# jbush001/RustNetworkStack

Measured on AMD Instinct MI355X. Metric: GiB/s device-resident Internet checksum, 1500B-packet batches, 1/2/4/8 GPUs, higher is better.
Workload: dtype u8

## Files before the change

### rustnetworkstack_amd/csrc/k_packed.hip

```cpp
#include "rns_launch.hpp"

#ifndef RNS_ROWS_DEEP_FROM
#define RNS_ROWS_DEEP_FROM 1024u
#endif
#ifndef RNS_TX_ROWS_DEEP_FROM
#define RNS_TX_ROWS_DEEP_FROM 1024u
#endif
#ifndef RNS_RX_ROWS_D
#define RNS_RX_ROWS_D 8
#endif

namespace rns {

constexpr bool kStreamNT = RNS_STREAM_NT != 0;

template <class Kernel>
static int launch_rows(const CsumArgs &a, uint32_t deep_from, hipStream_t st, Kernel kernel)
{
    return with_flags(
        [&](auto deep, auto buf) {
            return launch(kernel(std::integral_constant<int, deep() ? 16 : 8>{}, buf), dim3(waves64(a.n)), dim3(64), 0,
                          st, a);
        },
        a.len_hint >= deep_from, buf_ok(a));
}

int launch_stream_rx(const CsumArgs &a, hipStream_t st)
{
    return with_flags(
        [&](auto ack, auto buf) {
            if constexpr (ack())
                return launch(csum_stream_kernel<kStreamNT, buf()>, dim3(waves64(a.n)), dim3(64), 0, st, a);
            else
                return launch(csum_rows_rx_kernel<kStreamNT, buf(), RNS_RX_ROWS_D>, dim3(waves64(a.n)), dim3(64), 0, st,
                              a);
        },
        a.arena_bytes / a.n <= 128, buf_ok(a));
}

int dispatch_packed(const CsumArgs &a, const Shape &sh, hipStream_t st)
{
    const bool tiny = (sh.variant & ~16u) == 3u && sh.G == 4u && sh.U == 1u;
    if (a.align_mask >= 15u && !tiny)
        return launch_rows(a, RNS_ROWS_DEEP_FROM, st,
                           [](auto D, auto buf) { return csum_rows_kernel<kStreamNT, buf(), D()>; });
    const bool mixed = (sh.variant & 4u) != 0;
    if (!mixed && !tiny)
        return RNS_E_INVALID;
    const uint64_t batches = waves64(a.n);
    const uint64_t wpb = (mixed ? kMixedBlock<false> : kBlock) / 64;
    uint64_t blocks = (batches + wpb - 1) / wpb;
    if (sh.max_blocks != 0 && blocks > sh.max_blocks)
        blocks = sh.max_blocks;
    const dim3 grid(static_cast<uint32_t>(blocks)), block(mixed ? kMixedBlock<false> : kBlock);
    if (mixed)
        return with_flags(
            [&](auto nt, auto buf) {
                return launch(csum_mixed_kernel<false, nt(), buf(), false, false, false, true>, grid, block, 0, st, a);
            },
            (sh.variant & 2u) != 0, buf_ok(a));
    return with_flags(
        [&](auto buf, auto pf) {
            return launch(csum_rounds_kernel<4, 1, false, true, buf(), 1, true, pf()>, grid, block, 0, st, a);
        },
        buf_ok(a), (sh.variant & 16u) != 0);
}

int launch_fill_packed(const CsumArgs &a, hipStream_t st)
{
    return launch_rows(a, RNS_ROWS_DEEP_FROM, st,
                       [](auto D, auto buf) { return csum_rows_kernel<kStreamNT, buf(), D(), true>; });
}

int launch_tx_packed(const CsumArgs &a, hipStream_t st)
{
    return launch_rows(a, RNS_TX_ROWS_DEEP_FROM, st,
                       [](auto D, auto buf) { return csum_rows_tx_kernel<kStreamNT, buf(), D()>; });
}

int launch_strided_rx(const CsumArgs &a, hipStream_t st)
{
    constexpr int B = kStridedRxB;
    const dim3 grid(static_cast<uint32_t>((static_cast<uint64_t>(a.n) + 64 * B - 1) / (64 * B)));
    return with_flags([&](auto buf) { return launch(csum_strided_rx_kernel<buf(), B>, grid, dim3(64), 0, st, a); },
                      buf_ok(a));
}

// ... 2 lines not shown
```

### rustnetworkstack_amd/csrc/rns_checksum.hip

```cpp
#include <hip/hip_runtime.h>

#include <algorithm>
#include <cmath>
#include <cstdint>
#include <cstdio>

#include "rns_launch.hpp"

using namespace rns;

namespace {

__global__ __launch_bounds__(kBlock) void splitmix64_fill_kernel(uint8_t *buf, uint64_t nbytes, uint64_t seed)
{
    const uint64_t nwords = (nbytes + 7) / 8;
    const uint64_t stride = static_cast<uint64_t>(gridDim.x) * blockDim.x;
    for (uint64_t i = static_cast<uint64_t>(blockIdx.x) * blockDim.x + threadIdx.x; i < nwords; i += stride) {
        uint64_t z = seed + (i + 1) * 0x9E3779B97F4A7C15ull;
        z = (z ^ (z >> 30)) * 0xBF58476D1CE4E5B9ull;
        z = (z ^ (z >> 27)) * 0x94D049BB133111EBull;
        z = z ^ (z >> 31);
        if ((i + 1) * 8 <= nbytes) {
            reinterpret_cast<uint64_t *>(buf)[i] = z;
        } else {
// ... 115 lines not shown

#ifndef RNS_CHAIN_NT_FROM
#define RNS_CHAIN_NT_FROM 384u
#endif
bool chain_nt_from_hint(uint32_t frag_len_hint) { return (frag_len_hint ? frag_len_hint : 512u) >= RNS_CHAIN_NT_FROM; }
bool chain_nt_from_arena(uint64_t arena_bytes, uint32_t n_frags, double mean)
{
    const double frag_est = mean > 0.5 ? static_cast<double>(arena_bytes) / n_frags * (mean - 0.5) / mean : 0.0;
    return n_frags == 0 || frag_est >= RNS_CHAIN_NT_FROM;
}

bool chain_deep(uint32_t K, double mean) { return K >= 3 || (K == 2 && mean >= 2.0); }

template <bool FILL>
int chain_launch(CsumArgs &a, uint32_t frag_len_hint, hipStream_t stream)
{
    const double mean = chain_mean(a);
    a.chain_k = chain_pick_k(mean);
    if ((a.flags & RNS_FLAG_CHAIN_TX_PACKED) && mean <= 1.0 + kRunFrags)
        return launch_txrows<FILL>(a, stream);
    const bool runs = kChainRuns && (a.flags & RNS_FLAG_CHAIN_RUNS) && buf_ok(a);
    return launch_chain<FILL>(a, a.chain_k, chain_nt_from_hint(frag_len_hint), runs, chain_deep(a.chain_k, mean), stream);
}

constexpr uint64_t kRxGridCap = 4096;
dim3 stash_grid(uint64_t n, uint64_t arena_bytes, bool tiny_cap)
{
    constexpr int BLK = kMixedBlock<true>;
    uint64_t blocks = (waves64(n) + BLK / 64 - 1) / (BLK / 64);
    const bool cap = tiny_cap && arena_bytes / n <= 128;
    if (cap && blocks > kRxGridCap)
        blocks = kRxGridCap;
    return dim3(static_cast<uint32_t>(blocks));
}

bool misaligned(const void *p, uintptr_t mask) { return (reinterpret_cast<uintptr_t>(p) & mask) != 0; }

bool pool_rx_valid(const uint8_t *d_pool, uint32_t buf_log2, uint32_t min_log2, const uint32_t *d_buf_idx, uint32_t n_frags,
                   const uint32_t *d_blk_first, const uint16_t *d_len16, uint32_t n_pkts, const uint8_t *local_ipv4,
                   const uint8_t *local_ipv6, const uint8_t *d_status)
{
    return d_pool && buf_log2 >= min_log2 && buf_log2 <= kPoolMaxLog2 && d_blk_first && d_len16 && (!n_frags || d_buf_idx) &&
           n_pkts <= RNS_CHAIN_MAX_PACKETS && !misaligned(d_pool, 15) && rx_valid(d_status, local_ipv4, local_ipv6);
}

int pool_rx_verify(PoolRx &rx, bool &nt, const uint8_t *d_pool, uint64_t pool_bytes, uint32_t buf_log2,
                   const uint32_t *d_buf_idx, uint32_t n_frags, const uint32_t *d_blk_first, const uint16_t *d_len16,
                   uint32_t n_pkts, const uint8_t *local_ipv4, const uint8_t *local_ipv6, uint8_t *d_status, uint16_t *d_l4_sum,
                   void *stream)
{
    RNS_TRY(rns_rx_verify_pool_dev(d_pool, pool_bytes, buf_log2, d_buf_idx, n_frags, d_blk_first, d_len16, n_pkts, local_ipv4,
                                   local_ipv6, d_status, d_l4_sum, stream));
    rx = PoolRx{d_pool, pool_bytes, d_buf_idx, d_blk_first, d_len16, d_status, n_pkts, n_frags, buf_log2};
    nt = chain_nt_from_arena(pool_bytes, n_frags, static_cast<double>(n_frags) / n_pkts);
    return RNS_OK;
}

bool pool_tx_valid(const uint8_t *d_tx_pool, const uint32_t *d_free, uint32_t n_free, uint32_t cap, const uint32_t *d_ip_id_add,
                   const uint32_t *d_tx_blk_first, const uint8_t *d_tx_head_len8, const uint16_t *d_tx_pay_len16,
                   const uint32_t *d_tx_src, const uint32_t *d_count)
{
    return d_tx_pool && d_count && (!n_free || d_free) && (!cap || (d_tx_blk_first && d_tx_head_len8 && d_tx_pay_len16)) &&
           !misaligned(d_tx_pool, 15) && !misaligned(d_free, 3) && !misaligned(d_ip_id_add, 3) &&
           !misaligned(d_tx_blk_first, 3) && !misaligned(d_tx_pay_len16, 1) && !misaligned(d_tx_src, 3) &&
           !misaligned(d_count, 3);
}

void set_pool_tx(PoolTx &tx, uint8_t *d_tx_pool, uint64_t tx_pool_bytes, uint32_t buf_log2, const uint32_t *d_free,
                 uint32_t n_free, uint32_t cap, uint16_t ip_id_base, const uint32_t *d_ip_id_add, uint32_t *d_tx_blk_first,
                 uint8_t *d_tx_head_len8, uint16_t *d_tx_pay_len16, uint32_t *d_tx_src, uint32_t *d_count)
{
    tx = PoolTx{d_tx_pool, tx_pool_bytes >> buf_log2, d_free, d_ip_id_add, d_tx_blk_first, d_tx_head_len8, d_tx_pay_len16,
                d_tx_src, d_count, n_free, cap, ip_id_base, buf_log2};
}

int count_only(uint32_t *d_count, size_t bytes, void *stream)
{
    if (!d_count || misaligned(d_count, 3))
        return RNS_E_INVALID;
    RNS_TRY(check_device());
    return launch_fill32(d_count, bytes / 4, 0u, static_cast<hipStream_t>(stream));
}

}

extern "C" {

int rns_csum_batch_dev_cfg(const uint8_t *d_arena, uint64_t arena_bytes, const uint64_t *d_off,
                           const uint32_t *d_len, const uint16_t *d_seed, uint16_t *d_out, uint32_t n,
                           uint32_t flags, uint32_t variant, uint32_t lanes_per_packet, uint32_t unroll,
                           uint32_t max_blocks, uint32_t *d_bad, void *stream)
{
    return entry(n, d_off && d_len && d_out, d_arena, arena_bytes, flags, stream, [&](CsumArgs &a, hipStream_t st) {
        set_explicit(a, d_off, d_len);
        set_results(a, d_seed, d_out, d_bad);
        return dispatch<false>(a, variant, lanes_per_packet, unroll, max_blocks, st);
    });
}

int rns_csum_batch_dev(const uint8_t *d_arena, uint64_t arena_bytes, const uint64_t *d_off,
                       const uint32_t *d_len, const uint16_t *d_seed, uint16_t *d_out, uint32_t n,
                       uint32_t flags, uint32_t len_hint, uint32_t *d_bad, void *stream)
{
    const Shape sh = pick_shape(len_hint);
    return rns_csum_batch_dev_cfg(d_arena, arena_bytes, d_off, d_len, d_seed, d_out, n, flags, sh.variant, sh.G,
                                  sh.U, sh.max_blocks, d_bad, stream);
}

int rns_csum_batch_dev_off32(const uint8_t *d_arena, uint64_t arena_bytes, const uint32_t *d_off32,
                             const uint32_t *d_len, const uint16_t *d_seed, uint16_t *d_out, uint32_t n,
                             uint32_t flags, uint32_t len_hint, uint32_t *d_bad, void *stream)
{
    return entry(n, d_off32 && d_len && d_out, d_arena, arena_bytes, flags, stream, [&](CsumArgs &a, hipStream_t st) {
        a.off32 = d_off32;
        a.len = d_len;
        set_results(a, d_seed, d_out, d_bad);
        const Shape sh = pick_shape(len_hint);
        return dispatch<false>(a, sh.variant, sh.G, sh.U, sh.max_blocks, st);
    });
}

int rns_csum_batch_packed_dev(const uint8_t *d_arena, uint64_t arena_bytes, const uint64_t *d_blk_off,
                              const uint16_t *d_len16, uint32_t align_log2, const uint16_t *d_seed, uint16_t *d_out,
                              uint32_t n, uint32_t flags, uint32_t len_hint, uint32_t *d_bad, void *stream)
{
    return entry(n, d_blk_off && d_len16 && d_out && packed_align(align_log2, 0), d_arena, arena_bytes, flags, stream,
                 [&](CsumArgs &a, hipStream_t st) {
                     set_packed(a, d_blk_off, d_len16, align_log2);
                     set_results(a, d_seed, d_out, d_bad);
                     a.len_hint = len_hint;
                     Shape sh = pick_shape(len_hint);
                     if ((sh.variant & 5u) == 0)
                         sh = Shape{6u, 0u, 0u, 0u};
                     return dispatch_packed(a, sh, st);
                 });
}

int rns_csum_batch_strided_dev(const uint8_t *d_arena, uint64_t arena_bytes, uint64_t first_off,
                               uint64_t stride, uint32_t len, const uint16_t *d_seed, uint16_t *d_out,
                               uint32_t n, uint32_t flags, uint32_t *d_bad, void *stream)
{
    return entry(n, d_out && strided_fits(first_off, stride, n), d_arena, arena_bytes, flags, stream,
                 [&](CsumArgs &a, hipStream_t st) {
                     set_strided(a, first_off, stride);
                     set_results(a, d_seed, d_out, d_bad);
                     a.fixed_len = len;
                     if (len != 0 && len <= 64 && ((first_off + a.base_adjust) & 15) == 0 && (stride & 15) == 0)
                         return launch_strided_tiny(a, st);
                     const Shape sh = pick_shape(len);
                     return dispatch<true>(a, sh.variant, sh.G, sh.U, sh.max_blocks, st);
                 });
}

int rns_csum_chain_dev(const uint8_t *d_arena, uint64_t arena_bytes, const uint64_t *d_frag_off,
                       const uint32_t *d_frag_len, uint32_t n_frags, const uint32_t *d_first,
                       const uint16_t *d_seed, uint16_t *d_out, uint32_t n_pkts, uint32_t flags,
                       uint32_t frag_len_hint, uint16_t *d_frag_sums, uint32_t *d_bad, void *stream)
{
    (void)d_frag_sums;
    return entry(n_pkts, d_out && chain_valid(d_frag_off, d_frag_len, d_first, n_frags, n_pkts), d_arena, arena_bytes,
                 flags, stream, [&](CsumArgs &a, hipStream_t st) {
                     set_chain(a, d_frag_off, d_frag_len, d_first, n_frags);
                     set_results(a, d_seed, d_out, d_bad);
                     return chain_launch<false>(a, frag_len_hint, st);
                 });
}

int rns_csum_chain_fill_dev(uint8_t *d_arena, uint64_t arena_bytes, const uint64_t *d_frag_off,
                            const uint32_t *d_frag_len, uint32_t n_frags, const uint32_t *d_first,
                            const uint16_t *d_seed, const uint16_t *d_field, uint32_t field_off, uint16_t *d_out,
                            uint32_t n_pkts, uint32_t flags, uint32_t frag_len_hint, uint32_t *d_bad, void *stream)
{
    return entry(n_pkts, chain_valid(d_frag_off, d_frag_len, d_first, n_frags, n_pkts), d_arena, arena_bytes, flags,
                 stream, [&](CsumArgs &a, hipStream_t st) {
                     set_chain(a, d_frag_off, d_frag_len, d_first, n_frags);
                     set_results(a, d_seed, d_out, d_bad);
                     set_field(a, d_field, field_off);
                     return chain_launch<true>(a, frag_len_hint, st);
                 });
}

int rns_csum_fill_dev(uint8_t *d_arena, uint64_t arena_bytes, const uint64_t *d_off, const uint32_t *d_len,
                      const uint16_t *d_seed, const uint16_t *d_field, uint32_t field_off, uint16_t *d_out,
                      uint32_t n, uint32_t flags, uint32_t *d_bad, void *stream)
{
    return entry(n, d_off && d_len, d_arena, arena_bytes, flags, stream, [&](CsumArgs &a, hipStream_t st) {
        set_explicit(a, d_off, d_len);
        set_results(a, d_seed, d_out, d_bad);
        set_field(a, d_field, field_off);
        return launch_fill(a, stash_grid(n, arena_bytes, false), st);
    });
}

int rns_csum_fill_packed_dev(uint8_t *d_arena, uint64_t arena_bytes, const uint64_t *d_blk_off, const uint16_t *d_len16,
                             uint32_t align_log2, const uint16_t *d_seed, const uint16_t *d_field, uint32_t field_off,
                             uint16_t *d_out, uint32_t n, uint32_t flags, uint32_t len_hint, uint32_t *d_bad,
                             void *stream)
{
    return entry(n, d_blk_off && d_len16 && packed_align(align_log2, 4), d_arena, arena_bytes, flags, stream,
                 [&](CsumArgs &a, hipStream_t st) {
                     set_packed(a, d_blk_off, d_len16, align_log2);
// ... 475 lines not shown
                 d_head_blk_off && d_head_len8 && d_pay_blk_off && d_pay_len16 && packed_align(pay_align_log2, 4) &&
                     n <= RNS_CHAIN_MAX_PACKETS,
                 d_arena, arena_bytes, RNS_FLAG_COMPLEMENT, stream, [&](CsumArgs &a, hipStream_t st) {
                     a.head_blk_off = d_head_blk_off;
                     a.head_len8 = d_head_len8;
                     set_packed(a, d_pay_blk_off, d_pay_len16, pay_align_log2);
                     set_tx_status(a, d_status);
                     return launch_txrows<false, true, true>(a, st);
                 });
}

int rns_tx_fill_pool_dev(uint8_t *d_pool, uint64_t pool_bytes, uint32_t buf_log2, const uint32_t *d_buf_idx,
                         uint32_t n_frags, const uint32_t *d_blk_first, const uint8_t *d_head_len8,
                         const uint16_t *d_pay_len16, uint32_t n_pkts, uint8_t *d_status, void *stream)
{
    return entry(n_pkts,
                 buf_log2 >= kPoolTxMinLog2 && buf_log2 <= kPoolMaxLog2 && d_blk_first && d_head_len8 && d_pay_len16 &&
                     (!n_frags || d_buf_idx) && n_pkts <= RNS_CHAIN_MAX_PACKETS &&
                     (reinterpret_cast<uintptr_t>(d_pool) & 15) == 0,
                 d_pool, pool_bytes, RNS_FLAG_COMPLEMENT, stream, [&](CsumArgs &a, hipStream_t st) {
                     a.off32 = d_buf_idx;
                     a.n_frags = n_frags;
                     a.first = d_blk_first;
                     a.head_len8 = d_head_len8;
                     a.len16 = d_pay_len16;
                     a.align_mask = (1u << buf_log2) - 1u;
                     set_tx_status(a, d_status);
                     const double mean = chain_mean(a);
                     a.chain_k = chain_pick_k(mean);
                     return launch_tx_pool(a, a.chain_k, chain_nt_from_arena(pool_bytes, n_frags, mean), st);
                 });
}

int rns_tx_segment_dev(uint8_t *d_arena, uint64_t arena_bytes, const uint8_t *d_tmpl, uint32_t tmpl_stride,
                       const uint8_t *d_head_len8, const uint64_t *d_pay_off, const uint32_t *d_pay_len,
                       const uint16_t *d_mss, const uint64_t *d_head_off, const uint32_t *d_seg_first,
                       const uint32_t *d_blk_flow, uint32_t n_flows, uint32_t n_seg, uint8_t *d_status, void *stream)
{
    return entry(n_flows ? n_seg : 0u,
                 d_tmpl && tmpl_stride && d_head_len8 && d_pay_off && d_pay_len && d_mss && d_head_off && d_seg_first &&
                     d_blk_flow && n_seg <= RNS_CHAIN_MAX_PACKETS,
                 d_arena, arena_bytes, RNS_FLAG_COMPLEMENT, stream, [&](CsumArgs &a, hipStream_t st) {
                     a.tmpl = d_tmpl;
                     a.tmpl_stride = tmpl_stride;
                     a.n_flows = n_flows;
                     a.head_len8 = d_head_len8;
                     a.seg_pay_off = d_pay_off;
                     a.len = d_pay_len;
                     a.len16 = d_mss;
                     a.seg_head_off = d_head_off;
                     a.first = d_seg_first;
                     a.blk_flow = d_blk_flow;
                     set_tx_status(a, d_status);
                     return launch_tx_segment(a, arena_bytes / n_seg >= RNS_CHAIN_NT_FROM, st);
                 });
}

int rns_tx_fill_dev(uint8_t *d_arena, uint64_t arena_bytes, const uint64_t *d_off, const uint32_t *d_len,
                    uint32_t n, uint8_t *d_status, void *stream)
{
    return entry(n, d_off && d_len, d_arena, arena_bytes, RNS_FLAG_COMPLEMENT, stream, [&](CsumArgs &a, hipStream_t st) {
        set_explicit(a, d_off, d_len);
        set_tx_status(a, d_status);
        return launch_tx(a, stash_grid(n, arena_bytes, true), st);
    });
}

int rns_fill_splitmix64_dev(uint8_t *d_buf, uint64_t nbytes, uint64_t seed, void *stream)
{
    if (nbytes == 0)
        return RNS_OK;
    if (!d_buf || (reinterpret_cast<uintptr_t>(d_buf) & 7))
        return RNS_E_INVALID;
    RNS_TRY(check_device());
    const uint64_t words = (nbytes + 7) / 8;
    const uint32_t blocks = static_cast<uint32_t>(std::min<uint64_t>((words + kBlock - 1) / kBlock, 8192));
    hipLaunchKernelGGL(splitmix64_fill_kernel, dim3(blocks), dim3(kBlock), 0, static_cast<hipStream_t>(stream),
                       d_buf, nbytes, seed);
    return hip_status(hipGetLastError());
}

const char *rns_csum_shape_name(uint32_t len_hint)
{
    static const char *const names[] = {"csum_batch_kernel",     "csum_rounds_kernel",     "csum_batch_kernel[nt]",
                                        "csum_rounds_kernel[nt]", "csum_mixed_kernel",      "csum_mixed_kernel",
                                        "csum_mixed_kernel[nt]",  "csum_mixed_kernel[nt]"};
    static thread_local char buf[96];
    const Shape sh = pick_shape(len_hint);
    if (sh.variant & 4)
        std::snprintf(buf, sizeof(buf), "%s (size classes G/U 4/1 x 4 packets, 4/4, 16/4, 32/4, 64/4)", names[sh.variant & 7]);
    else
        std::snprintf(buf, sizeof(buf), "%s<G=%u,U=%u>%s%s", names[sh.variant & 7], sh.G, sh.U,
                      (sh.variant & 8) ? " all rounds in flight" : (sh.variant & 16) ? " descriptors prefetched" : "",
                      sh.max_blocks ? " grid-capped" : "");
    return buf;
}

const char *rns_build_info(void)
{
    return "rns_checksum abi=1 offload-arch=gfx950 kernels=csum_rows_kernel (packed form: 1 KiB rows per 64-packet "
           "region, owners capture two region prefixes and sum their own end chunk; fill mode), csum_rows_rx_kernel "
           "(packed receive verify: the rows plus each owner's header chunks loaded a group ahead), csum_stream_kernel "
           "(receive verify of ACK-sized arenas: owners load their datagrams whole), csum_strided_rx_kernel (receive "
           "verify of fixed-size slots: quad-coalesced rows), csum_rows_tx_kernel (packed transmit finalize through the "
           "rows), csum_txrows_kernel (transmit-shaped chains: packed payload rows + owner-loaded head fragments; "
           "head-fragment fill; whole finalize of NetBuffer chains with the heads written back from LDS), "
           "csum_strided_tiny_kernel "
           "(fixed-size packets <= 64 B at a fixed stride), csum_mixed_kernel (per-wave size-class sort; verify / fill / "
           "transmit-finalize stash modes), csum_rounds_kernel, csum_batch_kernel, csum_chain_kernel (one pass, "
           "per-fragment fold; head-fragment fill) (v_sad_u16 LE sums, v_dot4 BE sums past 128 KiB, wave64, DPP "
           "reductions)";
}

int rns_device_count(void)
{
    int n = 0;
    if (hipGetDeviceCount(&n) != hipSuccess) {
        (void)hipGetLastError();
        return 0;
    }
    return n;
}

}
```

### rustnetworkstack_amd/csrc/rns_k_stream.hpp

```cpp
#pragma once

#include "rns_k_chain.hpp"

namespace rns {

__device__ __forceinline__ uint4 keep_first(uint4 v, uint32_t c)
{
    const uint32_t bits = c * 8u;
    const uint64_t lo = ~0ull >> (64u - min(bits, 64u));
    const uint64_t hi = bits > 64u ? ~0ull >> ((128u - bits) & 63u) : 0ull;
    v.x &= static_cast<uint32_t>(lo);
    v.y &= static_cast<uint32_t>(lo >> 32);
    v.z &= static_cast<uint32_t>(hi);
    v.w &= static_cast<uint32_t>(hi >> 32);
    return v;
}

#ifndef RNS_STREAM_NT
#define RNS_STREAM_NT 1
#endif
#ifndef RNS_STREAM_OUT_AUX
#define RNS_STREAM_OUT_AUX 17
#endif
constexpr int kStreamD = 8;
constexpr int kStreamRxOcc = 6;

template <bool BUF>
__device__ __forceinline__ uint4 own_chunk(const CsumArgs &a, __amdgpu_buffer_rsrc_t rsrc, uint64_t recs, uint64_t off,
                                           uint32_t len, uint32_t i)
{
    const uint64_t o = off + 16u * i;
    return load16<BUF, false>(a, rsrc, o, 16u * i < len && o + 16 <= recs);
}

__device__ __forceinline__ void store_rx_status(const CsumArgs &a, uint64_t p, uint8_t stv, uint32_t l4_res)
{
    a.status[p] = stv;
    if (a.l4_out)
        a.l4_out[p] = static_cast<uint16_t>(l4_res);
}

template <bool NT, bool BUF>
__device__ __forceinline__ void wave_serial_sums(const CsumArgs &a, __amdgpu_buffer_rsrc_t rsrc, uint32_t lane,
                                                 uint64_t todo, uint64_t start, uint32_t len, uint32_t &mine)
{
    while (todo) {
        const uint32_t o = static_cast<uint32_t>(__builtin_ctzll(todo));
        todo &= todo - 1;
        const Pkt k = make_pkt(lane_u64(start, o), __builtin_amdgcn_readlane(len, o));
        uint32_t acc = 0;
        for (uint32_t cc = 0; cc < k.nch; cc += 64) {
            uint4 w[1];
            issue_pass<64, 1, NT, BUF, 1>(a, rsrc, k, cc + lane, w);
            mask_edges<64, 1, 1>(k, cc + lane, w);
            acc = sum_le<1, 1>(w, acc);
        }
        const uint32_t sum = group_allreduce<64>(acc);
        mine = lane == o ? sum : mine;
    }
}

struct PackedUnit {
    uint64_t p, q;
    bool live;
    uint32_t len, seed;
    uint64_t r0;
    uint32_t excl, total;
    __device__ __forceinline__ uint64_t start() const { return r0 + excl; }
    __device__ __forceinline__ bool ok(const CsumArgs &a) const
    {
        return start() <= a.arena_bytes && len <= a.arena_bytes - start();
    }
};

__device__ __forceinline__ PackedUnit packed_unit(const CsumArgs &a, uint32_t lane)
{
    PackedUnit u;
    const uint64_t base = static_cast<uint64_t>(blockIdx.x) * 64;
    u.p = base + lane;
    u.live = u.p < a.n;
    u.q = u.live ? u.p : a.n - 1;
    const uint32_t zero_v = __builtin_amdgcn_mbcnt_lo(0u, 0u);
    const uint64_t r0v = a.blk_off[(base >> 6) + zero_v];
    u.len = u.live ? static_cast<uint32_t>(a.len16[u.q]) : 0u;
    u.seed = (a.seed && u.live) ? static_cast<uint32_t>(a.seed[u.q]) : 0u;
    u.r0 = first_lane_u64(r0v) + a.base_adjust;
    const uint32_t pad = (u.len + a.align_mask) & ~a.align_mask;
    const uint32_t incl = wave_incl_scan(pad);
    u.excl = incl - pad;
    u.total = __builtin_amdgcn_readlane(incl, 63);
    return u;
}

template <bool BUF, bool MASKED, int N>
__device__ __forceinline__ uint32_t ack_unit_sum(const CsumArgs &a, __amdgpu_buffer_rsrc_t rsrc, uint64_t recs,
                                                 uint64_t start, uint32_t len, uint4 (&own)[N])
{
    static_assert(N >= 4, "four chunks hold an ACK-sized packet");
    uint32_t mine = 0;
#pragma unroll
    for (int i = 0; i < 4; ++i)
        own[i] = own_chunk<BUF>(a, rsrc, recs, start, len, i);
#pragma unroll
    for (int i = 0; i < 4; ++i) {
        uint4 x = own[i];
        if (16u * i + 16u > len)
            x = 16u * i < len ? keep_first(x, len - 16u * i) : make_uint4(0, 0, 0, 0);
        if constexpr (MASKED)
            own[i] = x;
        mine = sad4(x, mine);
    }
    return mine;
}

template <bool BUF, int N>
__device__ __forceinline__ uint32_t unaligned_head(const CsumArgs &a, __amdgpu_buffer_rsrc_t rsrc, uint64_t recs,
                                                   uint64_t start, uint32_t len, bool present, uint4 (&own)[N])
{
    const uint64_t b0 = start & ~15ull;
    const uint32_t s0 = static_cast<uint32_t>(start & 15);
#pragma unroll
    for (int i = 0; i < N; ++i)
        own[i] = own_chunk<BUF>(a, rsrc, recs, b0, present ? s0 + len : 0u, i);
#pragma unroll
    for (int i = 0; i < N; ++i) {
        const int lo = static_cast<int>(s0) - 16 * i, hi = static_cast<int>(s0 + len) - 16 * i;
        own[i] = make_uint4(keep_bytes(own[i].x, lo, hi, 0), keep_bytes(own[i].y, lo, hi, 4),
                            keep_bytes(own[i].z, lo, hi, 8), keep_bytes(own[i].w, lo, hi, 12));
    }
    return s0;
}

template <bool NT, bool BUF>
__global__ __launch_bounds__(64, kStreamRxOcc) void csum_stream_kernel(const CsumArgs a)
{
    constexpr int kNS = 4;
    constexpr uint32_t kTagShift = 17, kHead = 1u << 16, kEnd = 1u << 13, kStart = 1u << 12;
    __shared__ uint32_t tab[64];
    __shared__ uint32_t pend[64];
    __shared__ uint32_t pstart[64];
    __shared__ uint4 stash[64 * kNS];
    const uint32_t lane = threadIdx.x;
    const __amdgpu_buffer_rsrc_t rsrc = __builtin_amdgcn_make_buffer_rsrc(
        const_cast<uint8_t *>(a.arena), static_cast<short>(0), static_cast<int>(BUF ? buf_records(a) : 0), 0x00020000);
    const uint64_t recs = buf_records(a);
    const PackedUnit u = packed_unit(a, lane);
    const uint64_t p = u.p, r0 = u.r0;
    const uint32_t len = u.len, excl = u.excl, total = u.total;
    const bool live = u.live;
    uint32_t mine = 0;
    bool odd = false;

    if ((r0 & 15) == 0 && !__ballot(len > 64)) {
        const uint64_t start = u.start();
        const bool ok = u.ok(a);
        uint4 own[kNS + 1];
        mine = ack_unit_sum<BUF, true>(a, rsrc, recs, start, len, own);
        own[4] = make_uint4(0, 0, 0, 0);
        uint32_t l4_res = 0;
        const uint8_t stv = rx_finish<kNS + 1>(a, own, mine, 0u, len, false, false, live && ok && len != 0, l4_res);
        if (live)
            store_rx_status(a, p, stv, l4_res);
        return;
    }
    if ((r0 & 15) == 0) {
        const uint32_t la = static_cast<uint32_t>(reinterpret_cast<uintptr_t>(a.arena) + r0) & 127u;
        const uint32_t lead = la <= r0 ? la : 0u;
        const uint64_t rb = r0 - lead;
        const uint32_t nrows = (total + lead + 1023) >> 10;
        tab[lane] = 0xFFFFFFFFu;
        wave_lds_fence();
        uint32_t carry = 0;
        uint4 v[kStreamD];
        auto issue = [&](uint32_t k, uint4 &dst) {
// ... 190 lines not shown
```

### rustnetworkstack_amd/csrc/rns_k_txrows.hpp

```cpp
#pragma once

#include "rns_k_rows_tx.hpp"

namespace rns {

template <int NS>
__device__ __forceinline__ uint8_t chain_tx_head(const uint4 (&ch)[NS], uint32_t s, uint32_t hl, uint32_t L, bool odd,
                                                 bool present, uint32_t &ipv, uint32_t &l4f, uint32_t &hsum,
                                                 uint32_t &seed, uint32_t &hdr)
{
    ipv = 0;
    l4f = kNoField;
    hsum = 0;
    seed = 0;
    hdr = 0;
    if (!present)
        return RNS_TX_MALFORMED;
    uint32_t h[10];
    head40(ch, s, h);
    uint32_t field;
    bool v4;
    if (!tx_parse(h, L, hl, hdr, field, seed, v4))
        return RNS_TX_MALFORMED;
    const int lo = static_cast<int>(s);
// ... 39 lines not shown
    uint32_t f0 = 0, f1 = 0;
    uint32_t hl8 = 0, pl16 = 0;
    uint64_t hblk = 0, pblk = 0;
    if constexpr (CPT) {
        const uint64_t q = live ? p : a.n - 1;
        const uint64_t blk = (p >> 6) + __builtin_amdgcn_mbcnt_lo(0u, 0u);
        hblk = a.head_blk_off[blk];
        pblk = a.blk_off[blk];
        hl8 = live ? static_cast<uint32_t>(a.head_len8[q]) : 0u;
        pl16 = live ? static_cast<uint32_t>(a.len16[q]) : 0u;
        f1 = live ? (pl16 ? 2u : 1u) : 0u;
    } else {
        f0 = live ? a.first[p] : 0u;
        f1 = live ? a.first[p + 1] : 0u;
    }
    const bool rng_ok = CPT || (f0 <= f1 && f1 <= a.n_frags);
    const uint32_t nfr = live && rng_ok ? f1 - f0 : 0u;
    const uint32_t seed = (a.seed && live) ? static_cast<uint32_t>(a.seed[p]) : 0u;
    uint32_t fo = 0;
    if constexpr (FILL)
        fo = live ? (a.field ? static_cast<uint32_t>(a.field[p]) : a.field_off) : 0u;
    constexpr uint32_t kF = 1 + kRunFrags;
    uint64_t o[kF];
    uint32_t l[kF];
#pragma unroll
    for (uint32_t j = 0; j < kF; ++j) {
        o[j] = 0;
        l[j] = 0;
        if (!CPT && j < nfr) {
            o[j] = a.off[f0 + j] + a.base_adjust;
            l[j] = a.len[f0 + j];
        }
    }
    bool all_in = true, run = nfr <= kF;
    uint32_t plen = 0;
    uint64_t pbase = 0;
    if constexpr (CPT) {
        const uint32_t ppad = (pl16 + a.align_mask) & ~a.align_mask;
        const uint32_t hin = wave_incl_scan(hl8), pin = wave_incl_scan(ppad);
        pbase = lane_u64(pblk, 0) + a.base_adjust;
        o[0] = lane_u64(hblk, 0) + a.base_adjust + (hin - hl8);
        l[0] = hl8;
        o[1] = pbase + (pin - ppad);
        l[1] = pl16;
        plen = pl16;
        all_in = o[0] <= a.arena_bytes && hl8 <= a.arena_bytes - o[0] &&
                 (pl16 == 0 || (o[1] <= a.arena_bytes && pl16 <= a.arena_bytes - o[1]));
    }
#pragma unroll
    for (uint32_t j = 0; j < kF; ++j) {
        if (!CPT && j < nfr) {
            const bool in = o[j] <= a.arena_bytes && l[j] <= a.arena_bytes - o[j];
            all_in = all_in && in;
            if (j >= 1) {
                run = run && (j == 1 || (o[j] == o[j - 1] + l[j - 1] && !(l[j - 1] & 1u)));
                plen += l[j];
            }
        }
    }
    const uint32_t hl = l[0];
    bool bad = live && (!rng_ok || (nfr <= kF && !all_in));
    if constexpr (FILL)
        bad = bad || (live && (nfr == 0 || !(fo <= hl && hl - fo >= 2u)));
    if constexpr (FIN)
        bad = bad || (live && nfr == 0);
    const bool has_pay = live && !bad && plen != 0;
    const uint64_t po = o[1];
    const bool shape = !live || bad ||
                       (run && plen <= 0xFFFFu && (o[0] & 15u) + hl <= kHeadMax && (!has_pay || (po & 15u) == 0));
    const uint64_t pm = __ballot(has_pay);
    uint64_t r0 = 0;
    uint32_t rel = 0, c0 = 0, e = 0, total = 0;
    bool region = true;
    if constexpr (CPT) {
        region = !pm || (pbase & 15u) == 0;
        if (pm) {
            r0 = pbase;
            rel = static_cast<uint32_t>(po - pbase);
            const uint32_t last = 63u - static_cast<uint32_t>(__builtin_clzll(pm));
            total = __builtin_amdgcn_readlane(rel + ((plen + 15u) & ~15u), last);
            c0 = has_pay ? rel >> 4 : 0u;
            e = has_pay ? (rel + plen - 1u) >> 4 : 0u;
        }
    } else if (pm) {
        const uint32_t fl = static_cast<uint32_t>(__builtin_ctzll(pm));
        r0 = lane_u64(po, fl);
        const uint64_t rel64 = has_pay ? po - r0 : 0;
        const uint32_t pad = has_pay ? (plen + 15u) & ~15u : 0u;
        const bool near = rel64 < (1ull << 30);
        rel = static_cast<uint32_t>(rel64);
        const uint32_t end = has_pay && near ? rel + pad : 0u;
        const uint32_t incl = wave_incl_max(end);
        const uint32_t before = static_cast<uint32_t>(__shfl(static_cast<int>(incl), static_cast<int>(lane) - 1, 64));
        const bool asc = !has_pay || (near && (lane == 0 || rel >= before));
        total = __builtin_amdgcn_readlane(incl, 63);
        const uint32_t sum_pad = __builtin_amdgcn_readlane(wave_incl_scan(pad), 63);
        region = !__ballot(!asc) && total <= 2u * sum_pad + 4096u;
        c0 = has_pay ? rel >> 4 : 0u;
        e = has_pay ? (rel + plen - 1u) >> 4 : 0u;
    }
    const bool fast = !__ballot(!shape) && region;
    uint32_t res = 0;
    uint32_t fst = RNS_TX_MALFORMED, ipv = 0, l4f = kNoField;
    constexpr bool kRunWrite = FIN && RNS_TXFIN_RUNWRITE != 0;
    bool runw = false;
    uint64_t b0 = 0, r1 = 0;
    if constexpr (kRunWrite) {
        const uint64_t hend = o[0] + hl;
        const uint64_t pe = lane_below_u64(hend, lane);
        const bool contig = !live || (!bad && (CPT || lane == 0 || o[0] == pe));
        runw = fast && !__ballot(!contig);
        const uint32_t last = 63u - static_cast<uint32_t>(__builtin_clzll(__ballot(live)));
        b0 = first_lane_u64(o[0]) & ~15ull;
        r1 = lane_u64(hend, last);
    }
    __shared__ uint4 run_lds[kRunWrite ? 64u * kNH + 1u : 1u];
    if (fast) {
        const uint64_t hb = o[0] & ~15ull;
        const uint32_t hs = static_cast<uint32_t>(o[0] & 15u), span = live && !bad ? hs + hl : 0u;
        uint4 h[kNH];
#pragma unroll
        for (uint32_t i = 0; i < kNH; ++i)
            h[i] = own_chunk<BUF>(a, rsrc, recs, hb, span, i);
        uint32_t acc1 = 0;
        auto head = [&]() {
            uint32_t hsum = 0, sd = seed;
            if constexpr (kRunWrite) {
                if (runw) {
                    const uint32_t q = static_cast<uint32_t>((hb - b0) >> 4);
#pragma unroll
                    for (uint32_t i = 0; i < kNH; ++i)
                        if (16u * i < span)
                            run_lds[q + i] = h[i];
                }
            }
            if constexpr (FIN) {
                uint32_t hd;
                fst = chain_tx_head<kNH>(h, hs, hl, hl + plen, (o[0] & 1u) != 0, live && !bad, ipv, l4f, hsum, sd, hd);
            } else {
#pragma unroll
            for (uint32_t i = 0; i < 4; ++i) {
                const int lo = static_cast<int>(hs) - 16 * static_cast<int>(i), hi = static_cast<int>(span) - 16 * static_cast<int>(i);
                hsum = __builtin_amdgcn_sad_u16(keep_bytes(h[i].x, lo, hi, 0), 0, hsum);
                hsum = __builtin_amdgcn_sad_u16(keep_bytes(h[i].y, lo, hi, 4), 0, hsum);
                hsum = __builtin_amdgcn_sad_u16(keep_bytes(h[i].z, lo, hi, 8), 0, hsum);
                hsum = __builtin_amdgcn_sad_u16(keep_bytes(h[i].w, lo, hi, 12), 0, hsum);
            }
            }
            if constexpr (FILL) {
                const uint32_t w[16] = {h[0].x, h[0].y, h[0].z, h[0].w, h[1].x, h[1].y, h[1].z, h[1].w,
                                        h[2].x, h[2].y, h[2].z, h[2].w, h[3].x, h[3].y, h[3].z, h[3].w};
                const uint32_t q0 = hs + fo, q1 = q0 + 1u;
                uint32_t d0 = 0, d1 = 0;
#pragma unroll
                for (uint32_t d = 0; d < 16; ++d) {
                    d0 = (q0 >> 2) == d ? w[d] : d0;
                    d1 = (q1 >> 2) == d ? w[d] : d1;
                }
                const uint32_t b0 = (d0 >> ((q0 & 3u) * 8u)) & 0xffu, b1 = (d1 >> ((q1 & 3u) * 8u)) & 0xffu;
                hsum -= (live && !bad) ? (b0 << ((q0 & 1u) * 8u)) + (b1 << ((q1 & 1u) * 8u)) : 0u;
            }
            const uint32_t x = fold16(hsum);
            const uint32_t g = (o[0] & 1u) ? x : bswap16_u32(x);
            const uint32_t t = sd + g;
            acc1 = (t & 0xffff) + (t >> 16);
        };
        uint32_t mine = 0;
        if (pm) {
            mine = rows_region_sum<NT, BUF, D>(a, rsrc, recs, r0, total, c0, e, has_pay ? plen : 0u, nullptr, head);
        } else {
            head();
        }
        const uint32_t x = fold16(mine);
        const uint32_t t = acc1 + bswap16_u32(x);
        res = has_pay ? (t & 0xffff) + (t >> 16) : acc1;
    } else {
        uint32_t sd = seed, hd = 0;
        if constexpr (FIN) {
            uint32_t lt = 0;
            bool in = true;
            if constexpr (CPT) {
                lt = hl + plen;
// ... 153 lines not shown
```

### rustnetworkstack_amd/csrc/rns_kernels.hpp

```cpp
#pragma once

#include "rns_k_tcp_head.hpp"
#include "rns_k_common.hpp"
#include "rns_k_rounds.hpp"
#include "rns_k_mixed.hpp"
#include "rns_k_chain.hpp"
#include "rns_k_chain_rx.hpp"
#include "rns_k_pool_rx.hpp"
#include "rns_k_stream.hpp"
#include "rns_k_rows.hpp"
#include "rns_k_rows_rx.hpp"
#include "rns_k_rows_tx.hpp"
#include "rns_k_txrows.hpp"
#include "rns_k_pool_tx.hpp"
#include "rns_k_segment.hpp"
#include "rns_k_pool_view.hpp"
#include "rns_k_pool_place.hpp"
#include "rns_k_scan.hpp"
#include "rns_k_pool_txform.hpp"
#include "rns_k_args.hpp"
```

### rustnetworkstack_amd/csrc/rns_launch.hpp

```cpp
#pragma once

#include <type_traits>

#include "rns_kernels.hpp"

namespace rns {

inline int hip_status(hipError_t e) { return e == hipSuccess ? RNS_OK : RNS_E_HIP_BASE - static_cast<int>(e); }

struct Shape {
    uint32_t variant, G, U, max_blocks;
};

constexpr uint32_t kTinyVariant = 19u;
constexpr uint32_t kTinyGrid = 2048u;
inline Shape pick_shape(uint32_t len_hint)
{
    const uint32_t chunks = len_hint ? (len_hint + 15) / 16 + 1 : 96;
    if (chunks <= 8)
        return Shape{kTinyVariant, 4u, 1u, kTinyGrid};
    if (chunks <= 48)
        return Shape{4u, 0u, 0u, 0u};
    if (chunks <= 160)
        return Shape{6u, 0u, 0u, 0u};
    return Shape{2u, 64u, 4u, 0u};
}

inline int check_device()
{
    int n = 0;
    if (hipGetDeviceCount(&n) != hipSuccess || n <= 0) {
        (void)hipGetLastError();
        return RNS_E_NODEVICE;
    }
    return RNS_OK;
}

inline void set_arena(CsumArgs &a, const uint8_t *arena, uint64_t arena_bytes)
{
    const uintptr_t p = reinterpret_cast<uintptr_t>(arena);
    a.base_adjust = p & 15;
    a.arena = reinterpret_cast<const uint8_t *>(p - a.base_adjust);
    a.arena_bytes = arena_bytes + a.base_adjust;
}

inline bool buf_ok(const CsumArgs &a) { return buf_records(a) < kOobOffset; }

inline uint32_t waves64(uint64_t n) { return static_cast<uint32_t>((n + 63) / 64); }

template <class F>
int with_flags(F &&f)
{
    return f();
}
template <class F, class... Rest>
int with_flags(F &&f, bool b, Rest... rest)
{
    auto bind = [&](auto c) { return with_flags([&](auto... cs) { return f(c, cs...); }, rest...); };
    return b ? bind(std::true_type{}) : bind(std::false_type{});
}

template <uint32_t KM, uint32_t... More, class F>
int with_kmax(uint32_t K, F &&f)
{
    if constexpr (sizeof...(More) == 0)
        return f(std::integral_constant<uint32_t, KM>{});
    else
        return K <= KM ? f(std::integral_constant<uint32_t, KM>{}) : with_kmax<More...>(K, f);
}

inline int launch(void (*kernel)(const CsumArgs), dim3 grid, dim3 block, size_t lds, hipStream_t st, const CsumArgs &a)
{
    hipLaunchKernelGGL(kernel, grid, block, lds, st, a);
    return hip_status(hipGetLastError());
}

#define RNS_TRY(status)          \
    do {                         \
        if (int e = (status))    \
            return e;            \
    } while (0)
#define RNS_LAUNCH(kernel, grid, block, st, ...)                                      \
    do {                                                                              \
        hipLaunchKernelGGL(kernel, dim3(grid), dim3(block), 0, st, __VA_ARGS__);      \
        RNS_TRY(hip_status(hipGetLastError()));                                       \
    } while (0)

int launch_scan2_parts(uint2 *part, uint32_t nb, uint32_t *total2, hipStream_t st);
int launch_fill32(uint32_t *p, uint64_t n, uint32_t v, hipStream_t st);

template <class Classify, class Build>
int launch_build_seq(uint32_t *count, const BuildWork &w, uint64_t n, hipStream_t st, Classify classify, Build build)
{
    const uint32_t nb = static_cast<uint32_t>(scan_blocks(n));
    RNS_TRY(launch_fill32(count, 3, 0u, st));
    RNS_TRY(classify(nb));
    RNS_TRY(launch_scan2_parts(w.part_a, nb, nullptr, st));
    RNS_TRY(launch_scan2_parts(w.part_b, nb, nullptr, st));
    return build(nb);
}

template <bool S>
int dispatch(const CsumArgs &a, uint32_t variant, uint32_t G, uint32_t U, uint32_t max_blocks, hipStream_t st);
extern template int dispatch<false>(const CsumArgs &, uint32_t, uint32_t, uint32_t, uint32_t, hipStream_t);
extern template int dispatch<true>(const CsumArgs &, uint32_t, uint32_t, uint32_t, uint32_t, hipStream_t);
int launch_strided_tiny(const CsumArgs &a, hipStream_t st);
int dispatch_packed(const CsumArgs &a, const Shape &sh, hipStream_t st);
int launch_fill_packed(const CsumArgs &a, hipStream_t st);
int launch_stream_rx(const CsumArgs &a, hipStream_t st);
int launch_tx_packed(const CsumArgs &a, hipStream_t st);
int launch_strided_rx(const CsumArgs &a, hipStream_t st);
template <bool FILL>
int launch_chain(const CsumArgs &a, uint32_t K, bool nt, bool runs, bool deep, hipStream_t st);
extern template int launch_chain<false>(const CsumArgs &, uint32_t, bool, bool, bool, hipStream_t);
extern template int launch_chain<true>(const CsumArgs &, uint32_t, bool, bool, bool, hipStream_t);
template <bool FILL, bool FIN = false, bool CPT = false>
int launch_txrows(const CsumArgs &a, hipStream_t st);
extern template int launch_txrows<false, false, false>(const CsumArgs &, hipStream_t);
extern template int launch_txrows<true, false, false>(const CsumArgs &, hipStream_t);
extern template int launch_txrows<false, true, false>(const CsumArgs &, hipStream_t);
extern template int launch_txrows<false, true, true>(const CsumArgs &, hipStream_t);
int launch_rx_chain(const CsumArgs &a, uint32_t K, bool nt, hipStream_t st);
int launch_rx_pool(const CsumArgs &a, uint32_t K, bool nt, hipStream_t st);
int launch_tx_pool(const CsumArgs &a, uint32_t K, bool nt, hipStream_t st);
int launch_tx_segment(const CsumArgs &a, bool nt, hipStream_t st);
int launch_rx_place(const PlaceArgs &a, bool nt, hipStream_t st);
int launch_flow_update(const FlowArgs &a, hipStream_t st);
int launch_ack_build(const AckArgs &a, hipStream_t st);
int launch_flow_lists(const FlowArgs &a, uint32_t rec_dw, hipStream_t st);
int launch_conn_update(const FlowArgs &a, hipStream_t st);
int launch_ctl_build(const CtlArgs &a, hipStream_t st);
int launch_conn_close(const CloseArgs &a, hipStream_t st);
int launch_tx_plan(const PlanArgs &a, hipStream_t st);
int launch_rx_echo(const EchoArgs &a, bool nt, hipStream_t st);
int launch_rx_udp(const UdpArgs &a, bool nt, hipStream_t st);
int launch_tx_udp(const UdpTxArgs &a, hipStream_t st);
int launch_rx_listen(const ListenArgs &a, hipStream_t st);
int launch_fill(const CsumArgs &a, dim3 grid, hipStream_t st);
int launch_rx(const CsumArgs &a, dim3 grid, hipStream_t st);
int launch_tx(const CsumArgs &a, dim3 grid, hipStream_t st);

}
```

Baseline: 6741.

## Route explicit-descriptor checksums through row kernel when waves ascend contiguously

Adds a kernel for explicit offset/length descriptors. Each wave checks whether its 64 packets start at ascending 16-byte-aligned offsets in a compact region. If so, it sums them with the 1 KiB-row region path used by the packed form; otherwise it falls back to the size-class pass. The region-detection logic is factored out of the tx rows kernel so both paths share it. The aim is coalesced row loads instead of per-packet gathers for the default explicit entry points, at the cost of an extra ballot/scan prologue per wave and a divergent fallback.

```diff
diff --git a/rustnetworkstack_amd/csrc/k_explicit.hip b/rustnetworkstack_amd/csrc/k_explicit.hip
--- /dev/null
+++ b/rustnetworkstack_amd/csrc/k_explicit.hip
@@ -0,0 +1,15 @@
+#include "rns_launch.hpp"
+
+namespace rns {
+
+int launch_rows_explicit(const CsumArgs &a, uint32_t len_hint, bool nt, hipStream_t st)
+{
+    return with_flags(
+        [&](auto deep, auto buf, auto off32, auto NT) {
+            constexpr int D = deep() ? 16 : kExplicitShallowD;
+            return launch(csum_rows_explicit_kernel<NT(), buf(), D, off32()>, dim3(waves64(a.n)), dim3(64), 0, st, a);
+        },
+        len_hint >= RNS_ROWS_DEEP_FROM, buf_ok(a), a.off32 != nullptr, nt);
+}
+
+}
diff --git a/rustnetworkstack_amd/csrc/k_packed.hip b/rustnetworkstack_amd/csrc/k_packed.hip
--- a/rustnetworkstack_amd/csrc/k_packed.hip
+++ b/rustnetworkstack_amd/csrc/k_packed.hip
@@ -1,8 +1,5 @@
 #include "rns_launch.hpp"
 
-#ifndef RNS_ROWS_DEEP_FROM
-#define RNS_ROWS_DEEP_FROM 1024u
-#endif
 #ifndef RNS_TX_ROWS_DEEP_FROM
 #define RNS_TX_ROWS_DEEP_FROM 1024u
 #endif
diff --git a/rustnetworkstack_amd/csrc/rns_checksum.hip b/rustnetworkstack_amd/csrc/rns_checksum.hip
--- a/rustnetworkstack_amd/csrc/rns_checksum.hip
+++ b/rustnetworkstack_amd/csrc/rns_checksum.hip
@@ -221,6 +221,14 @@
     return launch_fill32(d_count, bytes / 4, 0u, static_cast<hipStream_t>(stream));
 }
 
+int explicit_launch(const CsumArgs &a, uint32_t len_hint, hipStream_t st)
+{
+    const Shape sh = pick_shape(len_hint);
+    if (sh.variant == kTinyVariant)
+        return dispatch<false>(a, sh.variant, sh.G, sh.U, sh.max_blocks, st);
+    return launch_rows_explicit(a, len_hint, (sh.variant & 2u) != 0, st);
+}
+
 }
 
 extern "C" {
@@ -241,9 +249,11 @@
                        const uint32_t *d_len, const uint16_t *d_seed, uint16_t *d_out, uint32_t n,
                        uint32_t flags, uint32_t len_hint, uint32_t *d_bad, void *stream)
 {
-    const Shape sh = pick_shape(len_hint);
-    return rns_csum_batch_dev_cfg(d_arena, arena_bytes, d_off, d_len, d_seed, d_out, n, flags, sh.variant, sh.G,
-                                  sh.U, sh.max_blocks, d_bad, stream);
+    return entry(n, d_off && d_len && d_out, d_arena, arena_bytes, flags, stream, [&](CsumArgs &a, hipStream_t st) {
+        set_explicit(a, d_off, d_len);
+        set_results(a, d_seed, d_out, d_bad);
+        return explicit_launch(a, len_hint, st);
+    });
 }
 
 int rns_csum_batch_dev_off32(const uint8_t *d_arena, uint64_t arena_bytes, const uint32_t *d_off32,
@@ -254,8 +264,7 @@
         a.off32 = d_off32;
         a.len = d_len;
         set_results(a, d_seed, d_out, d_bad);
-        const Shape sh = pick_shape(len_hint);
-        return dispatch<false>(a, sh.variant, sh.G, sh.U, sh.max_blocks, st);
+        return explicit_launch(a, len_hint, st);
     });
 }
 
@@ -897,16 +906,15 @@
 
 const char *rns_csum_shape_name(uint32_t len_hint)
 {
-    static const char *const names[] = {"csum_batch_kernel",     "csum_rounds_kernel",     "csum_batch_kernel[nt]",
-                                        "csum_rounds_kernel[nt]", "csum_mixed_kernel",      "csum_mixed_kernel",
-                                        "csum_mixed_kernel[nt]",  "csum_mixed_kernel[nt]"};
-    static thread_local char buf[96];
+    static thread_local char buf[192];
     const Shape sh = pick_shape(len_hint);
-    if (sh.variant & 4)
-        std::snprintf(buf, sizeof(buf), "%s (size classes G/U 4/1 x 4 packets, 4/4, 16/4, 32/4, 64/4)", names[sh.variant & 7]);
+    if (sh.variant != kTinyVariant)
+        std::snprintf(buf, sizeof(buf),
+                      "csum_rows_explicit_kernel<D=%d> (ordered 16-byte-aligned waves: 1 KiB rows; other waves: size classes "
+                      "G/U 4/1 x 4 packets, 4/4, 16/4, 32/4, 64/4%s)",
+                      len_hint >= RNS_ROWS_DEEP_FROM ? 16 : kExplicitShallowD, (sh.variant & 2) ? " [nt]" : "");
     else
-        std::snprintf(buf, sizeof(buf), "%s<G=%u,U=%u>%s%s", names[sh.variant & 7], sh.G, sh.U,
-                      (sh.variant & 8) ? " all rounds in flight" : (sh.variant & 16) ? " descriptors prefetched" : "",
+        std::snprintf(buf, sizeof(buf), "csum_rounds_kernel[nt]<G=%u,U=%u> descriptors prefetched%s", sh.G, sh.U,
                       sh.max_blocks ? " grid-capped" : "");
     return buf;
 }
@@ -914,7 +922,9 @@
 const char *rns_build_info(void)
 {
     return "rns_checksum abi=1 offload-arch=gfx950 kernels=csum_rows_kernel (packed form: 1 KiB rows per 64-packet "
-           "region, owners capture two region prefixes and sum their own end chunk; fill mode), csum_rows_rx_kernel "
+           "region, owners capture two region prefixes and sum their own end chunk; fill mode), csum_rows_explicit_kernel "
+           "(explicit descriptors: the rows for every wave whose 64 packets ascend at 16-byte starts, else the size "
+           "classes), csum_rows_rx_kernel "
            "(packed receive verify: the rows plus each owner's header chunks loaded a group ahead), csum_stream_kernel "
            "(receive verify of ACK-sized arenas: owners load their datagrams whole), csum_strided_rx_kernel (receive "
            "verify of fixed-size slots: quad-coalesced rows), csum_rows_tx_kernel (packed transmit finalize through the "
diff --git a/rustnetworkstack_amd/csrc/rns_k_rows_explicit.hpp b/rustnetworkstack_amd/csrc/rns_k_rows_explicit.hpp
--- /dev/null
+++ b/rustnetworkstack_amd/csrc/rns_k_rows_explicit.hpp
@@ -0,0 +1,52 @@
+#pragma once
+
+#include "rns_k_mixed.hpp"
+#include "rns_k_rows.hpp"
+
+namespace rns {
+
+constexpr int kExplicitOcc = 4;
+constexpr int kExplicitShallowD = 8;
+
+template <bool NT, bool BUF, int D, bool OFF32>
+__global__ __launch_bounds__(64, kExplicitOcc) void csum_rows_explicit_kernel(const CsumArgs a)
+{
+    const uint32_t lane = threadIdx.x;
+    const __amdgpu_buffer_rsrc_t rsrc = __builtin_amdgcn_make_buffer_rsrc(
+        const_cast<uint8_t *>(a.arena), static_cast<short>(0), static_cast<int>(BUF ? buf_records(a) : 0), 0x00020000);
+    const uint64_t recs = buf_records(a);
+    const uint64_t p = static_cast<uint64_t>(blockIdx.x) * 64 + lane;
+    const bool live = p < a.n;
+    const uint64_t q = live ? p : a.n - 1;
+    uint64_t off;
+    if constexpr (OFF32)
+        off = a.off32[q];
+    else
+        off = a.off[q];
+    if constexpr (BUF)
+        off = off > 0xFFFFFFFFull ? 0xFFFFFFFFull : off;
+    off = live ? off : 0;
+    uint32_t d_len = live ? a.len[q] : 0u;
+    uint64_t d_start = off + a.base_adjust;
+    const uint32_t d_seed = (a.seed && live) ? a.seed[p] : 0u;
+    const bool d_ok = d_start <= a.arena_bytes && d_len <= a.arena_bytes - d_start;
+    if (!d_ok || d_len == 0) {
+        d_len = 0;
+        d_start = 0;
+    }
+    const bool odd = d_start & 1, big = d_len > kNoWrapBytes;
+    const ExplicitRegion g = explicit_region(a, d_start, d_len, d_len != 0, lane);
+    uint32_t mine;
+    if (g.region) {
+        mine = rows_region_sum<RNS_STREAM_NT != 0, BUF, D>(a, rsrc, recs, g.r0, g.total, g.c0, g.e, d_len);
+    } else {
+        uint32_t pos;
+        mine = wave_class_pass<NT, BUF, kStashNone>(a, rsrc, d_start, d_len, 0xFFFFFFFFu, lane, nullptr, pos);
+    }
+    const uint16_t res = finalize_bits(mine, odd, big, d_seed, d_ok, a.flags);
+    if (live && a.out)
+        __builtin_nontemporal_store(res, a.out + p);
+    count_rejected(a, lane, live && !d_ok);
+}
+
+}
diff --git a/rustnetworkstack_amd/csrc/rns_k_stream.hpp b/rustnetworkstack_amd/csrc/rns_k_stream.hpp
--- a/rustnetworkstack_amd/csrc/rns_k_stream.hpp
+++ b/rustnetworkstack_amd/csrc/rns_k_stream.hpp
@@ -90,6 +90,39 @@
     u.excl = incl - pad;
     u.total = __builtin_amdgcn_readlane(incl, 63);
     return u;
+}
+
+struct ExplicitRegion {
+    uint64_t r0;
+    uint32_t rel, c0, e, total;
+    bool region;
+};
+
+__device__ __forceinline__ ExplicitRegion explicit_region(const CsumArgs &a, uint64_t start, uint32_t len, bool has,
+                                                          uint32_t lane)
+{
+    ExplicitRegion g{0, 0u, 0u, 0u, 0u, true};
+    const uint64_t pm = __ballot(has);
+    if (pm) {
+        const uint32_t fl = static_cast<uint32_t>(__builtin_ctzll(pm));
+        g.r0 = lane_u64(start, fl);
+        const uint64_t rel64 = has ? start - g.r0 : 0;
+        const uint32_t pad = has ? (len + 15u) & ~15u : 0u;
+        const bool near = rel64 < (1ull << 30);
+        g.rel = static_cast<uint32_t>(rel64);
+        const bool fits = len <= 0xFFFFu && (g.rel & 15u) == 0;
+        const uint32_t end = has && near ? g.rel + pad : 0u;
+        const uint32_t incl = wave_incl_max(end);
+        const uint32_t before = static_cast<uint32_t>(__shfl(static_cast<int>(incl), static_cast<int>(lane) - 1, 64));
+        const bool asc = !has || (near && fits && (lane == 0 || g.rel >= before));
+        g.total = __builtin_amdgcn_readlane(incl, 63);
+        const uint32_t sum_pad = __builtin_amdgcn_readlane(wave_incl_scan(pad), 63);
+        const bool r0_aligned = ((static_cast<uint32_t>(reinterpret_cast<uintptr_t>(a.arena)) + static_cast<uint32_t>(g.r0)) & 15u) == 0;
+        g.region = !__ballot(!asc) && r0_aligned && g.total <= 2u * sum_pad + 4096u;
+        g.c0 = has ? g.rel >> 4 : 0u;
+        g.e = has ? (g.rel + len - 1u) >> 4 : 0u;
+    }
+    return g;
 }
 
 template <bool BUF, bool MASKED, int N>
diff --git a/rustnetworkstack_amd/csrc/rns_k_txrows.hpp b/rustnetworkstack_amd/csrc/rns_k_txrows.hpp
--- a/rustnetworkstack_amd/csrc/rns_k_txrows.hpp
+++ b/rustnetworkstack_amd/csrc/rns_k_txrows.hpp
@@ -145,22 +145,13 @@
             c0 = has_pay ? rel >> 4 : 0u;
             e = has_pay ? (rel + plen - 1u) >> 4 : 0u;
         }
-    } else if (pm) {
-        const uint32_t fl = static_cast<uint32_t>(__builtin_ctzll(pm));
-        r0 = lane_u64(po, fl);
-        const uint64_t rel64 = has_pay ? po - r0 : 0;
-        const uint32_t pad = has_pay ? (plen + 15u) & ~15u : 0u;
-        const bool near = rel64 < (1ull << 30);
-        rel = static_cast<uint32_t>(rel64);
-        const uint32_t end = has_pay && near ? rel + pad : 0u;
-        const uint32_t incl = wave_incl_max(end);
-        const uint32_t before = static_cast<uint32_t>(__shfl(static_cast<int>(incl), static_cast<int>(lane) - 1, 64));
-        const bool asc = !has_pay || (near && (lane == 0 || rel >= before));
-        total = __builtin_amdgcn_readlane(incl, 63);
-        const uint32_t sum_pad = __builtin_amdgcn_readlane(wave_incl_scan(pad), 63);
-        region = !__ballot(!asc) && total <= 2u * sum_pad + 4096u;
-        c0 = has_pay ? rel >> 4 : 0u;
-        e = has_pay ? (rel + plen - 1u) >> 4 : 0u;
+    } else {
+        const ExplicitRegion g = explicit_region(a, po, plen, has_pay, lane);
+        r0 = g.r0;
+        total = g.total;
+        c0 = g.c0;
+        e = g.e;
+        region = g.region;
     }
     const bool fast = !__ballot(!shape) && region;
     uint32_t res = 0;
diff --git a/rustnetworkstack_amd/csrc/rns_kernels.hpp b/rustnetworkstack_amd/csrc/rns_kernels.hpp
--- a/rustnetworkstack_amd/csrc/rns_kernels.hpp
+++ b/rustnetworkstack_amd/csrc/rns_kernels.hpp
@@ -9,6 +9,7 @@
 #include "rns_k_pool_rx.hpp"
 #include "rns_k_stream.hpp"
 #include "rns_k_rows.hpp"
+#include "rns_k_rows_explicit.hpp"
 #include "rns_k_rows_rx.hpp"
 #include "rns_k_rows_tx.hpp"
 #include "rns_k_txrows.hpp"
diff --git a/rustnetworkstack_amd/csrc/rns_launch.hpp b/rustnetworkstack_amd/csrc/rns_launch.hpp
--- a/rustnetworkstack_amd/csrc/rns_launch.hpp
+++ b/rustnetworkstack_amd/csrc/rns_launch.hpp
@@ -45,6 +45,10 @@
 }
 
 inline bool buf_ok(const CsumArgs &a) { return buf_records(a) < kOobOffset; }
+
+#ifndef RNS_ROWS_DEEP_FROM
+#define RNS_ROWS_DEEP_FROM 1024u
+#endif
 
 inline uint32_t waves64(uint64_t n) { return static_cast<uint32_t>((n + 63) / 64); }
 
@@ -105,6 +109,7 @@
 extern template int dispatch<false>(const CsumArgs &, uint32_t, uint32_t, uint32_t, uint32_t, hipStream_t);
 extern template int dispatch<true>(const CsumArgs &, uint32_t, uint32_t, uint32_t, uint32_t, hipStream_t);
 int launch_strided_tiny(const CsumArgs &a, hipStream_t st);
+int launch_rows_explicit(const CsumArgs &a, uint32_t len_hint, bool nt, hipStream_t st);
 int dispatch_packed(const CsumArgs &a, const Shape &sh, hipStream_t st);
 int launch_fill_packed(const CsumArgs &a, hipStream_t st);
 int launch_stream_rx(const CsumArgs &a, hipStream_t st);
```

Result: no change. 6718 (-0.3%).
